# youngyoonii/mdistiller-ddp

Measured on AMD Instinct MI355X. Metric: images/sec (whole node) DKD ResNet32x4->ResNet8x4 CIFAR-100, higher is better.
Workload: dtype bf16; 1 GPU; model=DKD resnet32x4->resnet8x4, global_batch=64, per_gpu_batch=64, parallelism=dp1, graph=True, graph_comm=False, backend=auto, comm_backend=none, train_kernels=True, cfg=configs/cifar100/dkd/res32x4_res8x4.yaml

## Files before the change

mdistiller_ddp_amd/ops/csrc/conv_igemm.hip:

```cpp
#include "common.h"
#include "bnslot.h"
#include <stdlib.h>
#include <mutex>
#include <unordered_map>


namespace {

typedef __attribute__((ext_vector_type(8))) __bf16 bf16x8;
typedef __attribute__((ext_vector_type(4))) float f32x4;

constexpr int BK = 64;
constexpr int LDS_ROW = 72;

enum { LOAD_FAST = 0, LOAD_VEC8 = 1, LOAD_SCALAR = 2, LOAD_DGRAD_FAST = 3, LOAD_DGRAD_VEC8 = 4 };
enum { ACT_NONE = 0, ACT_RELU = 1, ACT_RELU6 = 2 };

struct ConvParams {
  const bf16_t* x;
  const bf16_t* w;
  const float* scale;
  const float* bias;
  const bf16_t* res;
  bf16_t* y;
// ... 835 lines not shown
      const int t = hdiv(s, p.dv_cb), cb = s - t * cin_blocks;
      th = pcv.nkw == 2 ? (t >> 1) : (pcv.nkw == 1 ? t : t / max(pcv.nkw, 1));
      tw = t - th * pcv.nkw;
      tap = (pcv.kh0 + p.par * th) * p.KW + pcv.kw0 + p.par * tw;
      c0 = cb * BK + chunk * 8;
      s = tap * cin_blocks + cb;
    } else if (FASTK) {
      tap = hdiv(s, p.dv_cb);
      c0 = (s - tap * cin_blocks) * BK + chunk * 8;
    } else {
      const int k0 = s * BK + chunk * 8;
      tap = hdiv(k0, p.dv_Cin);
      c0 = k0 - tap * p.Cin;
      kok = kok && k0 < p.K;
    }
    const int kh = hdiv(tap, p.dv_KW), kw = tap - kh * p.KW;
    const uint32_t abase = lds0 + (uint32_t)(buf * STAGE) + wave_off;
#pragma unroll
    for (int j = 0; j < AROWS; ++j) {
      int ih, iw;
      bool ok = kok;
      if (PAR) {
        ih = a_ih0[j] - th;
        iw = a_iw0[j] - tw;
        ok = ok && (unsigned)ih < (unsigned)p.H && (unsigned)iw < (unsigned)p.W;
      } else if (DGRAD) {
        const int nh = a_ih0[j] - kh, nw = a_iw0[j] - kw;
        ok = ok && nh >= 0 && nw >= 0;
        ih = nh; iw = nw;
        if (p.stride != 1) {
          ih = hdiv(max(nh, 0), p.dv_s);
          iw = hdiv(max(nw, 0), p.dv_s);
          ok = ok && ih * p.stride == nh && iw * p.stride == nw;
        }
        ok = ok && ih < p.H && iw < p.W;
      } else {
        ih = a_ih0[j] + kh;
        iw = a_iw0[j] + kw;
        ok = ok && (unsigned)ih < (unsigned)p.H && (unsigned)iw < (unsigned)p.W;
      }
      const bf16_t* src = ok ? p.x + (a_img[j] + (ih * p.W + iw) * p.ldx + c0) : zero;
      glds16(src, abase + (uint32_t)(j * 32 * 128));
    }
    const uint32_t bbase = abase + (uint32_t)(BM * 128);
#pragma unroll
    for (int j = 0; j < BLOADS; ++j) {
      const bf16_t* src = (live && b_ok[j]) ? b_row[j] + s * BK : zero;
      glds16(src, bbase + (uint32_t)(j * 32 * 128));
    }
  };

  f32x4 acc[MI][NI];
#pragma unroll
  for (int i = 0; i < MI; ++i)
#pragma unroll
    for (int j = 0; j < NI; ++j) acc[i][j] = (f32x4){0.f, 0.f, 0.f, 0.f};

  const int frow = lane & 15;
  const int swz = (frow >> 1) & 7;
  const int g4 = lane >> 4;
  auto compute = [&](int buf) {
    const char* As = smem + buf * STAGE;
    const char* Bs = As + BM * 128;
#pragma unroll
    for (int kk = 0; kk < 2; ++kk) {
      const int coff = ((kk * 4 + g4) ^ swz) * 16;
      bf16x8 af[MI], bfr[NI];
#pragma unroll
      for (int i = 0; i < MI; ++i)
        af[i] = *(const bf16x8*)(As + (wm * (BM / 2) + i * 16 + frow) * 128 + coff);
#pragma unroll
      for (int j = 0; j < NI; ++j)
        bfr[j] = *(const bf16x8*)(Bs + (wn * (BN / 2) + j * 16 + frow) * 128 + coff);
#pragma unroll
      for (int i = 0; i < MI; ++i)
#pragma unroll
        for (int j = 0; j < NI; ++j)
          acc[i][j] = __builtin_amdgcn_mfma_f32_16x16x32_bf16(af[i], bfr[j], acc[i][j], 0, 0, 0);
    }
  };

  const int n = s_end - s_begin;
  if constexpr (RING == 1) {
    for (int t = 0; t < n; ++t) {
      if (t) __syncthreads();
      issue(s_begin + t, 0);
      vm_wait_barrier<0>();
      compute(0);
    }
  } else {
#pragma unroll
    for (int s0 = 0; s0 < RING - 1; ++s0) issue(s_begin + s0, s0);
    stamp(p, 1);
    int cbuf = 0;
    for (int t = 0; t < n; ++t) {
      vm_wait_barrier<NL * (RING - 2)>();
      if (t == 0) stamp(p, 2);
      const int ibuf = cbuf == 0 ? RING - 1 : cbuf - 1;
      issue(s_begin + t + RING - 1, ibuf);
      compute(cbuf);
      cbuf = cbuf == RING - 1 ? 0 : cbuf + 1;
    }
  }
  vm_wait_barrier<0>();
  stamp(p, 3);
  conv_epilogue<BM, BN>(p, acc, smem, m0, n0, BM, pcv, PAR, pre);
  if (p.stamps != nullptr) {
    __syncthreads();
    stamp(p, 4);
  }
}

constexpr int HALO_BM = 128;
constexpr int HALO_PIECES = 7;
constexpr int HALO_PROWS = HALO_PIECES * 32;
constexpr int HALO1_PIECES = 8;
constexpr int HALO1_PROWS = HALO1_PIECES * 32;

template <int BN, int RING = 3>
struct HaloSmem {
  static constexpr int PATCH = HALO_PROWS * 128;
  static constexpr int BT = BN * 128;
  static constexpr int PIPE = 2 * PATCH + RING * BT;
  static constexpr int CTILE = ConvSmem<HALO_BM, BN>::CTILE;
  static constexpr int BYTES = PIPE > CTILE ? PIPE : CTILE;
};

template <int BN, bool FLIP, int RING = 3>
__global__ void __launch_bounds__(256) __attribute__((amdgpu_waves_per_eu((BN >= 128 || RING > 3) ? 1 : 2)))
conv_halo_kernel(const ConvParams p) {
  constexpr int BM = HALO_BM;
  constexpr int MI = BM / 32, NI = BN / 32;
  constexpr int BLOADS = (BN * 8 + 255) / 256;
  constexpr int PATCH = HaloSmem<BN, RING>::PATCH;
  constexpr int BT = HaloSmem<BN, RING>::BT;

  __shared__ __attribute__((aligned(16))) char smem[HaloSmem<BN, RING>::BYTES];
  typedef __attribute__((address_space(3))) char lds_char;
  const uint32_t lds0 = (uint32_t)(uintptr_t)(lds_char*)smem;

  const int tid = threadIdx.x, lane = tid & 63, wid = tid >> 6;
  const int wm = wid >> 1, wn = wid & 1;
  const int PB = p.hpb;
  const int m0 = blockIdx.x * PB;
  const int n0 = blockIdx.y * BN;
  const uint32_t wave_off = (uint32_t)__builtin_amdgcn_readfirstlane(wid) * 1024u;
  const bf16_t* const zero = (const bf16_t*)g_zero16;
  stamp(p, 0);

  const int W = p.W, H = p.H;
  const int IMGS = p.himgs;
  const int RH = p.hrows;
  const int PW = W + 2;
  const int PH = RH + 2;
  const int grow0 = hdiv(m0, p.dv_W);
  const int img0 = hdiv(grow0, p.dv_H);
  const int oh0 = grow0 - img0 * H;
  EpiPre<BM, BN, 256> pre;
  epi_prefetch(p, pre, m0, n0, PB, false);
  stamp(p, 5);

  const int trow = tid >> 3;
  const int chunk = (tid & 7) ^ (trow & 6);
  int p_src[HALO_PIECES];
  {
    const int P = IMGS * PH * PW;
#pragma unroll
    for (int j = 0; j < HALO_PIECES; ++j) {
      const int pr = 32 * j + trow;
      int off = -1;
      if (pr < P) {
        const int img = hdiv(pr, p.dv_PHPW);
        const int rem = pr - img * PH * PW;
        const int ir = hdiv(rem, p.dv_PW), ic = rem - ir * PW;
        const int n = img0 + img;
        const int ih = oh0 + ir - 1, iw = ic - 1;
        if (n < p.N && (unsigned)ih < (unsigned)H && (unsigned)iw < (unsigned)W)
          off = ((n * H + ih) * W + iw) * p.Cin;
      }
      p_src[j] = off;
    }
  }
  const bf16_t* b_row[BLOADS];
  bool b_ok[BLOADS];
#pragma unroll
  for (int j = 0; j < BLOADS; ++j) {
    const int co = n0 + trow + 32 * j;
    b_ok[j] = (trow + 32 * j < BN) && co < p.Cout;
    b_row[j] = p.w + (int64_t)(b_ok[j] ? co : 0) * p.Kp + chunk * 8;
  }

  stamp(p, 6);
  const int nchunks = p.Cin / BK;
  const int c_begin = blockIdx.z * p.steps_per_split;
  const int c_end = min(nchunks, c_begin + p.steps_per_split);
  const int nsteps = (c_end - c_begin) * 9;

  auto issue_b = [&](int step, int bbuf) {
    const bool live = step < nsteps;
    const int st = live ? step : 0;
    const int cc = c_begin + st / 9, tap = st - (st / 9) * 9;
    const int wtap = FLIP ? 8 - tap : tap;
    const uint32_t base = lds0 + 2 * PATCH + (uint32_t)(bbuf * BT) + wave_off;
#pragma unroll
    for (int j = 0; j < BLOADS; ++j) {
      const bf16_t* src = (live && b_ok[j]) ? b_row[j] + wtap * p.Cin + cc * BK : zero;
      glds16(src, base + (uint32_t)(j * 32 * 128));
    }
  };
  auto issue_piece = [&](int cc, int pbuf, int j) {
    const bool live = cc < c_end;
    const int off = p_src[j];
    const bf16_t* src = (live && off >= 0) ? p.x + off + cc * BK + chunk * 8 : zero;
    glds16(src, lds0 + (uint32_t)(pbuf * PATCH) + wave_off + (uint32_t)(j * 32 * 128));
  };

  f32x4 acc[MI][NI];
#pragma unroll
  for (int i = 0; i < MI; ++i)
#pragma unroll
    for (int j = 0; j < NI; ++j) acc[i][j] = (f32x4){0.f, 0.f, 0.f, 0.f};

  const int frow = lane & 15;
  const bool p8 = W == 8 && p.perm8 != 0;
  const int g4 = lane >> 4;
  int a_prow[MI];
#pragma unroll
  for (int i = 0; i < MI; ++i) {
    int ml = wm * (BM / 2) + i * 16 + (p8 ? perm8(frow) : frow);
    if (ml >= PB) ml = 0;
    const int lr = hdiv(ml, p.dv_W), c = ml - lr * W;
    const int img = hdiv(lr, p.dv_RH), r = lr - img * RH;
    a_prow[i] = (img * PH + r) * PW + c;
  }
  const int bswz = frow & 6;

  auto compute = [&](int pbuf, int bbuf, int tap) {
    const char* Ps = smem + pbuf * PATCH;
    const char* Bs = smem + 2 * PATCH + bbuf * BT;
    const int kh = tap / 3, kw = tap - (tap / 3) * 3;
    const int toff = kh * PW + kw;
#pragma unroll
    for (int kk = 0; kk < 2; ++kk) {
      const int q = kk * 4 + g4;
      bf16x8 af[MI], bfr[NI];
#pragma unroll
      for (int i = 0; i < MI; ++i) {
        const int pr = a_prow[i] + toff;
        af[i] = *(const bf16x8*)(Ps + pr * 128 + ((q ^ (pr & 6)) * 16));
      }
#pragma unroll
      for (int j = 0; j < NI; ++j)
        bfr[j] = *(const bf16x8*)(Bs + (wn * (BN / 2) + j * 16 + frow) * 128 + ((q ^ bswz) * 16));
#pragma unroll
      for (int i = 0; i < MI; ++i)
#pragma unroll
        for (int j = 0; j < NI; ++j)
          acc[i][j] = __builtin_amdgcn_mfma_f32_16x16x32_bf16(af[i], bfr[j], acc[i][j], 0, 0, 0);
    }
  };

#pragma unroll
  for (int j = 0; j < HALO_PIECES; ++j) issue_piece(c_begin, 0, j);
#pragma unroll
  for (int s0 = 0; s0 < RING - 1; ++s0) issue_b(s0, s0);
  stamp(p, 1);
  int pbuf = 0, bbuf = 0, step = 0;
  for (int cc = c_begin; cc < c_end; ++cc) {
#pragma unroll
    for (int tap = 0; tap < 9; ++tap) {
      if (RING == 3) {
        if (tap == 0) vm_wait_barrier<BLOADS>();
        else if (tap == 1) vm_wait_barrier<BLOADS + 1>();
        else if (tap <= 7) vm_wait_barrier<BLOADS + 2>();
        else vm_wait_barrier<BLOADS + 1>();
      } else {
        if (tap == 0) vm_wait_barrier<2 * BLOADS>();
        else vm_wait_barrier<(RING - 2) * BLOADS>();
      }
      if (step == 0) stamp(p, 2);
      int nb = bbuf + RING - 1;
      if (nb >= RING) nb -= RING;
      issue_b(step + RING - 1, nb);
      if (tap < HALO_PIECES) issue_piece(cc + 1, pbuf ^ 1, tap);
      compute(pbuf, bbuf, tap);
      bbuf = bbuf == RING - 1 ? 0 : bbuf + 1;
      ++step;
    }
    pbuf ^= 1;
  }
  vm_wait_barrier<0>();
  stamp(p, 3);
  conv_epilogue<BM, BN>(p, acc, smem, m0, n0, PB, ParClass{}, false, pre, p8);
  if (p.stamps != nullptr) {
    __syncthreads();
    stamp(p, 4);
  }
}

template <int BN>
struct Halo1Smem {
  static constexpr int PATCH = HALO1_PROWS * 128;
  static constexpr int BT = BN * 128;
  static constexpr int RING = (81920 - PATCH) / BT > 9 ? 9 : (81920 - PATCH) / BT;
  static constexpr int PIPE = PATCH + RING * BT;
  static constexpr int CTILE = ConvSmem<HALO_BM, BN>::CTILE;
  static constexpr int BYTES = PIPE > CTILE ? PIPE : CTILE;
};

template <int BN, bool FLIP>
__global__ void __launch_bounds__(256) __attribute__((amdgpu_waves_per_eu(2)))
conv_halo1_kernel(const ConvParams p) {
  constexpr int BM = HALO_BM;
  constexpr int MI = BM / 32, NI = BN / 32;
  constexpr int BLOADS = (BN * 8 + 255) / 256;
  constexpr int PATCH = Halo1Smem<BN>::PATCH;
  constexpr int BT = Halo1Smem<BN>::BT;
  constexpr int RING = Halo1Smem<BN>::RING;

  __shared__ __attribute__((aligned(16))) char smem[Halo1Smem<BN>::BYTES];
  typedef __attribute__((address_space(3))) char lds_char;
  const uint32_t lds0 = (uint32_t)(uintptr_t)(lds_char*)smem;

  const int tid = threadIdx.x, lane = tid & 63, wid = tid >> 6;
  const int wm = wid >> 1, wn = wid & 1;
  const int PB = p.hpb;
  const int m0 = blockIdx.x * PB;
  const int n0 = blockIdx.y * BN;
  const uint32_t wave_off = (uint32_t)__builtin_amdgcn_readfirstlane(wid) * 1024u;
  const bf16_t* const zero = (const bf16_t*)g_zero16;

  const int W = p.W, H = p.H;
  const int IMGS = p.himgs;
  const int RH = p.hrows;
  const int PW = W + 2;
  const int PH = RH + 2;
  const int grow0 = hdiv(m0, p.dv_W);
  const int img0 = hdiv(grow0, p.dv_H);
  const int oh0 = grow0 - img0 * H;
  EpiPre<BM, BN, 256> pre;
  epi_prefetch(p, pre, m0, n0, PB, false);

  const int trow = tid >> 3;
  const int chunk = (tid & 7) ^ (trow & 6);
  int p_src[HALO1_PIECES];
  {
    const int P = IMGS * PH * PW;
#pragma unroll
    for (int j = 0; j < HALO1_PIECES; ++j) {
      const int pr = 32 * j + trow;
      int off = -1;
      if (pr < P) {
        const int img = hdiv(pr, p.dv_PHPW);
        const int rem = pr - img * PH * PW;
        const int ir = hdiv(rem, p.dv_PW), ic = rem - ir * PW;
        const int n = img0 + img;
        const int ih = oh0 + ir - 1, iw = ic - 1;
        if (n < p.N && (unsigned)ih < (unsigned)H && (unsigned)iw < (unsigned)W)
          off = ((n * H + ih) * W + iw) * p.Cin;
      }
      p_src[j] = off;
    }
  }
  const bf16_t* b_row[BLOADS];
  bool b_ok[BLOADS];
#pragma unroll
  for (int j = 0; j < BLOADS; ++j) {
    const int co = n0 + trow + 32 * j;
    b_ok[j] = (trow + 32 * j < BN) && co < p.Cout;
    b_row[j] = p.w + (int64_t)(b_ok[j] ? co : 0) * p.Kp + chunk * 8;
  }

  const int c_begin = 0, c_end = 1;
  const int nsteps = 9;

  auto issue_b = [&](int step, int bbuf) {
    const bool live = step < nsteps;
    const int st = live ? step : 0;
    const int cc = c_begin + st / 9, tap = st - (st / 9) * 9;
    const int wtap = FLIP ? 8 - tap : tap;
    const uint32_t base = lds0 + PATCH + (uint32_t)(bbuf * BT) + wave_off;
#pragma unroll
    for (int j = 0; j < BLOADS; ++j) {
      const bf16_t* src = (live && b_ok[j]) ? b_row[j] + wtap * p.Cin + cc * BK : zero;
      glds16(src, base + (uint32_t)(j * 32 * 128));
    }
  };
  auto issue_piece = [&](int cc, int pbuf, int j) {
    const bool live = cc < c_end;
    const int off = p_src[j];
    const bf16_t* src = (live && off >= 0) ? p.x + off + cc * BK + chunk * 8 : zero;
    glds16(src, lds0 + (uint32_t)(pbuf * PATCH) + wave_off + (uint32_t)(j * 32 * 128));
  };

  f32x4 acc[MI][NI];
#pragma unroll
  for (int i = 0; i < MI; ++i)
#pragma unroll
    for (int j = 0; j < NI; ++j) acc[i][j] = (f32x4){0.f, 0.f, 0.f, 0.f};

  const int frow = lane & 15;
  const bool p8 = W == 8 && p.perm8 != 0;
  const int g4 = lane >> 4;
  int a_prow[MI];
#pragma unroll
  for (int i = 0; i < MI; ++i) {
    int ml = wm * (BM / 2) + i * 16 + (p8 ? perm8(frow) : frow);
    if (ml >= PB) ml = 0;
    const int lr = hdiv(ml, p.dv_W), c = ml - lr * W;
    const int img = hdiv(lr, p.dv_RH), r = lr - img * RH;
    a_prow[i] = (img * PH + r) * PW + c;
  }
  const int bswz = frow & 6;

  auto compute = [&](int pbuf, int bbuf, int tap) {
    const char* Ps = smem + pbuf * PATCH;
    const char* Bs = smem + PATCH + bbuf * BT;
    const int kh = tap / 3, kw = tap - (tap / 3) * 3;
    const int toff = kh * PW + kw;
#pragma unroll
    for (int kk = 0; kk < 2; ++kk) {
      const int q = kk * 4 + g4;
      bf16x8 af[MI], bfr[NI];
#pragma unroll
      for (int i = 0; i < MI; ++i) {
        const int pr = a_prow[i] + toff;
        af[i] = *(const bf16x8*)(Ps + pr * 128 + ((q ^ (pr & 6)) * 16));
      }
#pragma unroll
      for (int j = 0; j < NI; ++j)
        bfr[j] = *(const bf16x8*)(Bs + (wn * (BN / 2) + j * 16 + frow) * 128 + ((q ^ bswz) * 16));
#pragma unroll
      for (int i = 0; i < MI; ++i)
#pragma unroll
        for (int j = 0; j < NI; ++j)
          acc[i][j] = __builtin_amdgcn_mfma_f32_16x16x32_bf16(af[i], bfr[j], acc[i][j], 0, 0, 0);
    }
  };

#pragma unroll
  for (int j = 0; j < HALO1_PIECES; ++j) issue_piece(c_begin, 0, j);
#pragma unroll
  for (int s0 = 0; s0 < RING - 1; ++s0) issue_b(s0, s0);
#pragma unroll
  for (int tap = 0; tap < 9; ++tap) {
    vm_wait_barrier<(RING - 2) * BLOADS>();
    issue_b(tap + RING - 1, (tap + RING - 1) % RING);
    compute(0, tap % RING, tap);
  }
  vm_wait_barrier<0>();
  conv_epilogue<BM, BN>(p, acc, smem, m0, n0, PB, ParClass{}, false, pre, p8);
}

__global__ void __launch_bounds__(256) conv_splitk_epilogue(const ConvParams p, int splits) {
  const int64_t total = (int64_t)p.M * p.Cout;
  if ((p.Cout & 7) == 0) {
    const int64_t t8 = total >> 3;
    for (int64_t i = blockIdx.x * (int64_t)blockDim.x + threadIdx.x; i < t8;
         i += (int64_t)gridDim.x * blockDim.x) {
      float v[8] = {0.f, 0.f, 0.f, 0.f, 0.f, 0.f, 0.f, 0.f};
      for (int z = 0; z < splits; ++z) {
        const float* src = p.partial + (int64_t)z * total + i * 8;
        const float4 lo = *(const float4*)src, hi = *(const float4*)(src + 4);
        v[0] += lo.x; v[1] += lo.y; v[2] += lo.z; v[3] += lo.w;
        v[4] += hi.x; v[5] += hi.y; v[6] += hi.z; v[7] += hi.w;
      }
      const int m = (int)((i * 8) / p.Cout);
      const int co = (int)(i * 8 - (int64_t)m * p.Cout);
      float sc[8], bi[8];
      load_scale_bias8(p, co, sc, bi);
      epilogue_store8(p, m, co, v, sc, bi);
    }
    return;
  }
  for (int64_t i = blockIdx.x * (int64_t)blockDim.x + threadIdx.x; i < total;
       i += (int64_t)gridDim.x * blockDim.x) {
    float a = 0.f;
    for (int z = 0; z < splits; ++z) a += p.partial[(int64_t)z * total + i];
    const int m = (int)(i / p.Cout);
    const int co = (int)(i - (int64_t)m * p.Cout);
    epilogue_store(p, m, co, a);
  }
}

bool halo_geometry(ConvParams& p, int max_rows, int cap = HALO_BM) {
  if (p.KH != 3 || p.KW != 3 || p.stride != 1 || p.pad != 1) return false;
  if (p.Ho != p.H || p.Wo != p.W || p.Cin % BK || p.Kp != 9 * p.Cin) return false;
  if (p.W > HALO_BM) return false;
  int imgs = 1, rows = 0;
  if (p.H * p.W <= cap) {
    imgs = cap / (p.H * p.W);
    while (imgs > 1 && imgs * (p.H + 2) * (p.W + 2) > max_rows) --imgs;
    rows = p.H;
  } else {
    for (int r = cap / p.W; r >= 1; --r)
      if (p.H % r == 0 && (r + 2) * (p.W + 2) <= max_rows) { rows = r; break; }
  }
  if (rows <= 0 || imgs * (rows + 2) * (p.W + 2) > max_rows) return false;
  const int pb = imgs * rows * p.W;
  if (4 * pb < 3 * cap && !(p.H * p.W <= HALO_BM)) return false;
  p.hrows = rows;
  p.himgs = imgs;
  p.hpb = pb;
  make_hdiv((uint32_t)p.W, p.dv_W);
  make_hdiv((uint32_t)p.H, p.dv_H);
  make_hdiv((uint32_t)(p.W + 2), p.dv_PW);
  make_hdiv((uint32_t)((rows + 2) * (p.W + 2)), p.dv_PHPW);
  make_hdiv((uint32_t)rows, p.dv_RH);
  return true;
}

bool halo_eligible(ConvParams& p) {
  static const bool on = [] {
    const char* e = getenv("MDA_CONV_HALO");
    return !(e && e[0] == '0');
  }();
  if (!on) return false;
  return halo_geometry(p, p.Cin == BK ? HALO1_PROWS : HALO_PROWS);
}

bool grouped_bn_fit() {
  static const bool on = [] {
    const char* e = getenv("MDA_GROUPED_BN");
    return !(e && e[0] == '0');
  }();
  return on;
}

bool use_halo1() {
  static const bool on = [] {
    const char* e = getenv("MDA_CONV_HALO1");
    return !(e && e[0] == '0');
  }();
  return on;
}

int reg1x1_min_m() {
  static const int v = [] {
    const char* e = getenv("MDA_REG1X1_MIN_M");
    return e ? atoi(e) : 32768;
  }();
  return v;
}

bool use_xcd_remap() {
  static const bool on = [] {
    const char* e = getenv("MDA_CONV_XCD");
    return !(e && e[0] == '0');
  }();
  return on;
}

bool use_krot() {
  static const bool on = [] {
    const char* e = getenv("MDA_CONV_KROT");
    return e && e[0] == '1';
  }();
  return on;
}

bool use_par_dgrad() {
  static const bool on = [] {
    const char* e = getenv("MDA_DGRAD_PARITY");
    return !(e && e[0] == '0');
  }();
  return on;
}

int halo_ring() {
  static const int v = [] {
    const char* e = getenv("MDA_HALO_RING");
    return e ? atoi(e) : 3;
  }();
  return v;
}

int ring1_max() {
  static const int v = [] {
    const char* e = getenv("MDA_GLDS_RING1_MAX");
    return e ? atoi(e) : 4;
  }();
  return v;
}

bool use_glds() {
  static const bool on = [] {
    const char* e = getenv("MDA_CONV_GLDS");
    return !(e && e[0] == '0');
  }();
  return on;
}

#define DLAUNCH(K, G, B, S, ST, P) hipLaunchKernelGGL(K, G, B, S, ST, P)

template <int BM, int BN>
int launch_tile(const ConvParams& p, int mode, int splits, hipStream_t st) {
  const int ny = p.cout_g < p.Cout ? (p.Cout / p.cout_g) * ((p.cout_g + BN - 1) / BN)
                                   : (p.Cout + BN - 1) / BN;
  dim3 grid((p.M + BM - 1) / BM, ny, splits);
  if (p.cout_g < p.Cout && (mode == LOAD_SCALAR || !use_glds())) return (int)hipErrorInvalidValue;
  const bool reg1x1 = p.KH == 1 && p.KW == 1 && p.cout_g >= p.Cout &&
                      (p.M >= reg1x1_min_m() || p.Kp <= 4 * BK) &&
                      (mode == LOAD_FAST || mode == LOAD_VEC8);
  if (mode != LOAD_SCALAR && use_glds() && !reg1x1 && p.steps_per_split <= ring1_max()) {
    if (mode == LOAD_FAST)
      DLAUNCH((conv_glds_kernel<BM, BN, LOAD_FAST, 1>), grid, dim3(256), 0, st, p);
    else if (mode == LOAD_VEC8)
      DLAUNCH((conv_glds_kernel<BM, BN, LOAD_VEC8, 1>), grid, dim3(256), 0, st, p);
    else if (mode == LOAD_DGRAD_FAST)
      DLAUNCH((conv_glds_kernel<BM, BN, LOAD_DGRAD_FAST, 1>), grid, dim3(256), 0, st, p);
    else
      DLAUNCH((conv_glds_kernel<BM, BN, LOAD_DGRAD_VEC8, 1>), grid, dim3(256), 0, st, p);
    return (int)hipGetLastError();
  }
  if (mode != LOAD_SCALAR && use_glds() && !reg1x1) {
    if (mode == LOAD_FAST)
      DLAUNCH((conv_glds_kernel<BM, BN, LOAD_FAST>), grid, dim3(256), 0, st, p);
    else if (mode == LOAD_VEC8)
      DLAUNCH((conv_glds_kernel<BM, BN, LOAD_VEC8>), grid, dim3(256), 0, st, p);
    else if (mode == LOAD_DGRAD_FAST)
      DLAUNCH((conv_glds_kernel<BM, BN, LOAD_DGRAD_FAST>), grid, dim3(256), 0, st, p);
    else
      DLAUNCH((conv_glds_kernel<BM, BN, LOAD_DGRAD_VEC8>), grid, dim3(256), 0, st, p);
    return (int)hipGetLastError();
  }
  if (mode == LOAD_FAST)
    DLAUNCH((conv_fwd_kernel<BM, BN, LOAD_FAST>), grid, dim3(256), 0, st, p);
  else if (mode == LOAD_VEC8)
    DLAUNCH((conv_fwd_kernel<BM, BN, LOAD_VEC8>), grid, dim3(256), 0, st, p);
  else if (mode == LOAD_DGRAD_FAST)
    DLAUNCH((conv_fwd_kernel<BM, BN, LOAD_DGRAD_FAST>), grid, dim3(256), 0, st, p);
  else if (mode == LOAD_DGRAD_VEC8)
    DLAUNCH((conv_fwd_kernel<BM, BN, LOAD_DGRAD_VEC8>), grid, dim3(256), 0, st, p);
  else
    DLAUNCH((conv_fwd_kernel<BM, BN, LOAD_SCALAR>), grid, dim3(256), 0, st, p);
  return (int)hipGetLastError();
}

}

uint64_t* g_stamps = nullptr;

MDA_API int mda_conv_set_stamps(void* buf) {
  g_stamps = (uint64_t*)buf;
  return 0;
}

MDA_API int mda_conv_plan(int64_t M, int64_t Cout, int64_t Kp, int64_t* tile, int64_t* splits) {
  static const int64_t target = [] {
    const char* e = getenv("MDA_CONV_TARGET");
    return e ? (int64_t)atoi(e) : (int64_t)256;
  }();
  int bn = Cout <= 32 ? 32 : (Cout <= 64 ? 64 : 128);
  int bm = 128;
  auto blocks = [&](int bm_, int bn_) { return ((M + bm_ - 1) / bm_) * ((Cout + bn_ - 1) / bn_); };
  int64_t steps = Kp / BK;
  if (steps <= ring1_max() && bn == 128) bn = 64;
  if (blocks(bm, bn) < target && bn == 128) bn = 64;
  if (blocks(bm, bn) < target) bm = 64;
  int64_t nb = blocks(bm, bn);
  int64_t sp = 1;
  while (nb * sp < target && steps / (sp * 2) >= 4 && sp < 8) sp *= 2;
  *tile = bm * 1000 + bn;
  *splits = sp;
  return 0;
}

extern "C" int mda_conv1x1_stream_try(const void* x, const void* w, const float* scale,
                                      const float* bias, const void* res, void* y, void* preact,
                                      void* slot, int64_t N, int64_t H, int64_t W, int64_t K,
                                      int64_t Kp, int64_t Ho, int64_t Wo, int64_t Cout,
                                      int64_t stride, int64_t act, hipStream_t st);

namespace {

void glds_prep(ConvParams& p) {
  static const int perm8_on = [] {
    const char* e = getenv("MDA_HALO_PERM8");
    return (e && e[0] == '0') ? 0 : 1;
  }();
  p.perm8 = perm8_on;
  p.xcd = use_xcd_remap() ? 1 : 0;
  p.krot = use_krot() ? 1 : 0;
  make_hdiv((uint32_t)std::max(p.Cin, 1), p.dv_Cin);
  make_hdiv((uint32_t)std::max(p.KW, 1), p.dv_KW);
  make_hdiv((uint32_t)std::max(p.Cin / BK, 1), p.dv_cb);
  make_hdiv((uint32_t)std::max(p.Ho * p.Wo, 1), p.dv_HoWo);
  make_hdiv((uint32_t)std::max(p.Wo, 1), p.dv_Wo);
  make_hdiv((uint32_t)std::max(p.stride, 1), p.dv_s);
}

int dispatch(ConvParams& p, int mode, int64_t tile, int64_t splits, hipStream_t st, int halo = 0) {
  if (p.Kp % BK || p.Kp < p.K) return (int)hipErrorInvalidValue;
  if (p.ldx <= 0) p.ldx = p.Cin;
  if (p.cout_g <= 0) p.cout_g = p.Cout;
  if (p.KH == 1 && p.KW == 1 && p.pad == 0 && p.cout_g >= p.Cout && p.ldx == p.Cin &&
      p.bnb_slot == nullptr && p.stats_part == nullptr && p.stamps == nullptr &&
      (mode == LOAD_FAST || mode == LOAD_VEC8 ||
       ((mode == LOAD_DGRAD_FAST || mode == LOAD_DGRAD_VEC8) && p.stride == 1))) {
    const bool fwd = mode == LOAD_FAST || mode == LOAD_VEC8;
    const int rc = mda_conv1x1_stream_try(p.x, p.w, p.scale, p.bias, p.res, p.y, p.preact,
                                          p.stats_slot, p.N, p.H, p.W, p.Cin, p.Kp, p.Ho, p.Wo,
                                          p.Cout, fwd ? p.stride : 1, p.act, st);
    if (rc != -1) return rc;
  }
  glds_prep(p);
  if (p.cout_g < p.Cout) {
    if (p.Cout % p.cout_g || p.ldx != p.Cin * (p.Cout / p.cout_g) || p.cout_g % 8 || p.Cin % 8)
      return (int)hipErrorInvalidValue;
    halo = 0;
    p.par = 0;
  }
  const int64_t xb = (int64_t)p.N * p.H * p.W * p.ldx * 2, wb = (int64_t)p.Cout * p.Kp * 2;
  if (xb >= ((int64_t)1 << 31) || wb >= ((int64_t)1 << 31) || (int64_t)p.M * p.Cout >= ((int64_t)1 << 31))
    return (int)hipErrorInvalidValue;
  p.x_bytes = (int)xb;
  p.w_bytes = (int)wb;
  if (tile == 0 || splits == 0) mda_conv_plan(p.M, p.Cout, p.Kp, &tile, &splits);
  if (splits > 1 && p.partial == nullptr) return (int)hipErrorInvalidValue;
  if (p.cout_g < p.Cout && grouped_bn_fit()) {
    const int cg = p.cout_g;
    int best = (int)(tile % 1000), best_pad = (cg + best - 1) / best * best;
    for (int bn : {128, 64, 32}) {
      const int pad = (cg + bn - 1) / bn * bn;
      if (pad * 8 <= cg * 9) { best = bn; best_pad = pad; break; }
      if (pad < best_pad) { best = bn; best_pad = pad; }
    }
    tile = tile / 1000 * 1000 + best;
  }
  int rc;
  if (p.x2 != nullptr && (halo || p.par <= 1 || splits != 1 || p.cin2 % BK || p.cls2 < 0 ||
                          p.cls2 >= p.par * p.par))
    return MDA_NOT_SERVED;
  if (halo) {
    const int nchunks = p.Cin / BK;
    if (!(nchunks == 1 && splits == 1 && use_halo1()) &&
        p.himgs * (p.hrows + 2) * (p.W + 2) > HALO_PROWS)
      halo = 0;
  }
  if (halo) {
    const int nchunks = p.Cin / BK;
    p.steps_per_split = (int)((nchunks + splits - 1) / splits);
    const int bn = p.Cout <= 32 ? 32 : 64;
    dim3 grid((p.M + p.hpb - 1) / p.hpb, (p.Cout + bn - 1) / bn, (int)splits);
    if (nchunks == 1 && splits == 1 && use_halo1()) {
      if (bn == 32) {
        if (halo == 2) DLAUNCH((conv_halo1_kernel<32, true>), grid, dim3(256), 0, st, p);
        else DLAUNCH((conv_halo1_kernel<32, false>), grid, dim3(256), 0, st, p);
      } else {
        if (halo == 2) DLAUNCH((conv_halo1_kernel<64, true>), grid, dim3(256), 0, st, p);
        else DLAUNCH((conv_halo1_kernel<64, false>), grid, dim3(256), 0, st, p);
      }
    } else {
      const int64_t nblocks = (int64_t)grid.x * grid.y * grid.z;
// ... 332 lines not shown
```

Baseline: 85740 images/s.

## Restructure halo1 conv weight pipeline into fixed 6-slot, three-tap phases

Replaces the halo1 kernel's per-tap rolling weight ring, sized to fill LDS, with a fixed six-slot ring consumed in three phases of three taps, each phase separated by a full barrier. The smaller LDS footprint is asserted to fit two blocks per CU, aiming at better occupancy and fewer per-tap barrier waits. The cost is coarser overlap: the last three taps' loads are issued only after the first phase finishes, and each phase ends with a full drain. Timing stamps are also added, and they only run when stamps are enabled.

```diff
diff --git a/mdistiller_ddp_amd/ops/csrc/conv_igemm.hip b/mdistiller_ddp_amd/ops/csrc/conv_igemm.hip
--- a/mdistiller_ddp_amd/ops/csrc/conv_igemm.hip
+++ b/mdistiller_ddp_amd/ops/csrc/conv_igemm.hip
@@ -1161,8 +1161,8 @@
 struct Halo1Smem {
   static constexpr int PATCH = HALO1_PROWS * 128;
   static constexpr int BT = BN * 128;
-  static constexpr int RING = (81920 - PATCH) / BT > 9 ? 9 : (81920 - PATCH) / BT;
-  static constexpr int PIPE = PATCH + RING * BT;
+  static constexpr int PIPE = PATCH + 2 * 3 * BT;
+  static_assert(PIPE <= 81920, "two blocks per CU");
   static constexpr int CTILE = ConvSmem<HALO_BM, BN>::CTILE;
   static constexpr int BYTES = PIPE > CTILE ? PIPE : CTILE;
 };
@@ -1175,7 +1175,6 @@
   constexpr int BLOADS = (BN * 8 + 255) / 256;
   constexpr int PATCH = Halo1Smem<BN>::PATCH;
   constexpr int BT = Halo1Smem<BN>::BT;
-  constexpr int RING = Halo1Smem<BN>::RING;
 
   __shared__ __attribute__((aligned(16))) char smem[Halo1Smem<BN>::BYTES];
   typedef __attribute__((address_space(3))) char lds_char;
@@ -1188,6 +1187,7 @@
   const int n0 = blockIdx.y * BN;
   const uint32_t wave_off = (uint32_t)__builtin_amdgcn_readfirstlane(wid) * 1024u;
   const bf16_t* const zero = (const bf16_t*)g_zero16;
+  stamp(p, 0);
 
   const int W = p.W, H = p.H;
   const int IMGS = p.himgs;
@@ -1199,6 +1199,7 @@
   const int oh0 = grow0 - img0 * H;
   EpiPre<BM, BN, 256> pre;
   epi_prefetch(p, pre, m0, n0, PB, false);
+  stamp(p, 5);
 
   const int trow = tid >> 3;
   const int chunk = (tid & 7) ^ (trow & 6);
@@ -1230,6 +1231,7 @@
     b_row[j] = p.w + (int64_t)(b_ok[j] ? co : 0) * p.Kp + chunk * 8;
   }
 
+  stamp(p, 6);
   const int c_begin = 0, c_end = 1;
   const int nsteps = 9;
 
@@ -1300,15 +1302,27 @@
 #pragma unroll
   for (int j = 0; j < HALO1_PIECES; ++j) issue_piece(c_begin, 0, j);
 #pragma unroll
-  for (int s0 = 0; s0 < RING - 1; ++s0) issue_b(s0, s0);
-#pragma unroll
-  for (int tap = 0; tap < 9; ++tap) {
-    vm_wait_barrier<(RING - 2) * BLOADS>();
-    issue_b(tap + RING - 1, (tap + RING - 1) % RING);
-    compute(0, tap % RING, tap);
-  }
+  for (int t = 0; t < 6; ++t) issue_b(t, t);
+  stamp(p, 1);
+  vm_wait_barrier<3 * BLOADS>();
+  stamp(p, 2);
+#pragma unroll
+  for (int tap = 0; tap < 3; ++tap) compute(0, tap, tap);
   vm_wait_barrier<0>();
+#pragma unroll
+  for (int t = 0; t < 3; ++t) issue_b(6 + t, t);
+#pragma unroll
+  for (int tap = 3; tap < 6; ++tap) compute(0, tap, tap);
+  vm_wait_barrier<0>();
+#pragma unroll
+  for (int tap = 6; tap < 9; ++tap) compute(0, tap - 6, tap);
+  vm_wait_barrier<0>();
+  stamp(p, 3);
   conv_epilogue<BM, BN>(p, acc, smem, m0, n0, PB, ParClass{}, false, pre, p8);
+  if (p.stamps != nullptr) {
+    __syncthreads();
+    stamp(p, 4);
+  }
 }
 
 __global__ void __launch_bounds__(256) conv_splitk_epilogue(const ConvParams p, int splits) {
```

Result: no change. 85990 images/s (median of 2 runs) (+0.3%).
